# indrajeetadityaroy9/vit-bias-aware-structural-distillation

Measured on AMD Instinct MI355X. Metric: images/sec BASD train step, DeiT-T student / ViT-B teacher bs=256, higher is better.
Workload: dtype bf16

## Files before the change

### include/basd_hip.h

```cpp
#ifndef BASD_HIP_H
#define BASD_HIP_H

#include <stddef.h>
#include <stdint.h>

#ifdef __cplusplus
extern "C" {
#endif

#define BASD_OK 0
#define BASD_ERR_SHAPE 1
#define BASD_ERR_LAUNCH 2
#define BASD_ERR_WORKSPACE 3
#define BASD_ERR_DTYPE 4

#define BASD_STATUS_NONCONVERGED 1
#define BASD_STATUS_NONFINITE 2
#define BASD_STATUS_RANK0 4

#define BASD_DTYPE_F32 0
#define BASD_DTYPE_BF16 1
#define BASD_DTYPE_F64 2

#define BASD_JACOBI_MAX_COLS 256
// ... 30 lines not shown
                    int32_t* status, void* stream);

int basd_mp_rank(const float* evals, int batch, int n, int64_t rows, int d, int cap,
                 int32_t* ranks, int32_t* status, void* stream);

int basd_flag_if_exceeds_f64(const double* values, int64_t n, double tol, int bit, int32_t* status, void* stream);

int basd_angle_weights(const float* sigma, const float* sw, const float* log_temp, int E, int L, int D,
                       int unnormalised, float* d2, float* pre, float* weights, float* coef, void* stream);

int64_t basd_angle_weights_bwd_workspace_bytes(int E, int D, int D_s);
int basd_angle_weights_bwd(const float* g_w, const float* g_pre_out, const float* weights, const float* d2,
                           const float* log_temp, const float* t_seed, const float* v_s, const double* lam_s,
                           const float* proj_s, int E, int L, int D, int D_s, float* g_log_temp, float* w_tok,
                           void* workspace, int64_t workspace_bytes, void* stream);

int64_t basd_selector_frames_workspace_bytes(int n, int D);
int basd_selector_frames(const double* unc, const double* csum, int n, int64_t m_rows, int D, int with_ranks,
                         int32_t* ranks, float* sigma, double* lam, float* v, int32_t* status, void* workspace,
                         int64_t workspace_bytes, void* stream);

int64_t basd_selector_weights_workspace_bytes(int E, int L, int D);
int basd_selector_weights(const float* v_s, const int32_t* ranks, const float* vm_t, const float* sw,
                          const float* log_temp, int E, int L, int D, float* weights, float* pre, float* d2,
                          float* t_seed, int32_t* status, void* workspace, int64_t workspace_bytes, void* stream);

int basd_mix_tokens(const void* const* x_layers, int x_dtype, int L, int E,
                    const float* w, int64_t elems, int64_t per_batch, int64_t batch_stride,
                    float* out, void* stream);

int basd_procrustes_prep(const void* s, int s_dtype, int64_t s_batch_stride, const float* t, const float* imp,
                         int B, int N_s, int N_t, int D_s, int D_t,
                         float* s_w, float* t_w, float* a, float* tr, void* stream);

int basd_mix_grad_dots(const void* const* x_layers, int x_dtype, int L, int E,
                       const float* g, int64_t elems, int64_t per_batch, int64_t batch_stride,
                       double* dots, void* stream);

int basd_bgemm_f64(const void* a, int a_dtype, int64_t a_stride, int lda, int trans_a,
                   const void* b, int b_dtype, int64_t b_stride, int ldb, int trans_b,
                   void* c, int c_dtype, int64_t c_stride, int ldc,
                   int batch, int M, int N, int K, int symmetric, void* stream);
int basd_bgemm_f64_masked(const void* a, int a_dtype, int64_t a_stride, int lda, int trans_a,
                          const void* b, int b_dtype, int64_t b_stride, int ldb, int trans_b,
                          void* c, int c_dtype, int64_t c_stride, int ldc,
                          int batch, int M, int N, int K, int symmetric, const int32_t* skip, void* stream);

int basd_gemm_bf16(const void* x, const void* w, const void* bias, void* y, int64_t M, int N, int K,
                   int epilogue, int tile_run, void* stream);

int basd_gemm_bf16x3_f32(const void* x, const void* w3, float* y, int64_t M, int N, int K, void* stream);

int basd_gemm_bf16_gelu_fwd(const void* x, const void* w, const void* bias, void* pre, void* y, int64_t M, int N,
                            int K, int tile_run, void* stream);
int basd_gemm_bf16_gelu_bwd(const void* dy, const void* wt, const void* pre, void* dpre, int64_t M, int N, int K,
                            int tile_run, void* stream);

int basd_wgrad_bf16(const void* dy, const void* x, int64_t M, int N, int K, float* dw, float* db,
                    void* stream);

int64_t basd_wgrad_workspace_bytes(int64_t M, int N, int K);
int basd_wgrad_bf16_ws(const void* dy, const void* x, int64_t M, int N, int K, float* dw, float* db,
                       void* workspace, int64_t workspace_bytes, void* stream);

int basd_layernorm_fwd_bf16(const void* x, const float* gamma, const float* beta, int64_t rows, int D,
                            float eps, void* y, float* mean, float* rstd, void* stream);
// ... 105 lines not shown
```

### vit-bias-aware-structural-distillation_amd/_native.py

```python
from __future__ import annotations

import contextlib
import ctypes
import os
import subprocess

import torch

_HERE = os.path.dirname(os.path.abspath(__file__))
LIB_PATH = os.environ.get("BASD_LIB") or os.path.join(_HERE, "libbasd_hip.so")
CSRC = os.path.join(_HERE, "csrc")

DTYPE_F32, DTYPE_BF16, DTYPE_F64 = 0, 1, 2
JACOBI_LDS_BYTES = 163840

EXPORTS = (
    "basd_version", "basd_last_error", "basd_token_gram", "basd_token_gram_bf16x3", "basd_gram_f32_centred", "basd_pchol_f64", "basd_jacobi_svd",
    "basd_mp_rank", "basd_flag_if_exceeds_f64", "basd_angle_weights", "basd_ce_uwso",
    "basd_procrustes_workspace_bytes", "basd_procrustes_fwd", "basd_procrustes_bwd_side",
    "basd_procrustes_bwd_workspace_bytes", "basd_procrustes_bwd", "basd_angle_weights_bwd_workspace_bytes",
    "basd_angle_weights_bwd", "basd_mix_tokens", "basd_procrustes_prep", "basd_mix_grad_dots",
    "basd_sf_adamw_step", "basd_lerp", "basd_transpose_bf16_table", "basd_bgemm_f64", "basd_trinv_f64", "basd_bgemm_f64_masked", "basd_trinv_f64_masked", "basd_pchol_f64_masked", "basd_wgrad_bf16", "basd_wgrad_workspace_bytes", "basd_wgrad_bf16_ws", "basd_gemm_bf16",
    "basd_gemm_bf16_gelu_fwd", "basd_gemm_bf16_gelu_bwd", "basd_gemm_bf16x3_f32", "basd_layernorm_fwd_bf16", "basd_layernorm_bwd_bf16",
    "basd_cls_importance_bf16", "basd_add_layernorm_fwd_bf16", "basd_procrustes_bwd_rows", "basd_attention_fwd_bf16", "basd_attention_fwd_qmean_bf16", "basd_attention_bwd_bf16",
    "basd_split_bf16x2_table", "basd_split_patches_bf16x2", "basd_gemm_f32x3", "basd_attention_fwd_f32x3",
    "basd_add_layernorm_fwd_f32", "basd_selector_frames_workspace_bytes", "basd_selector_frames",
    "basd_selector_weights_workspace_bytes", "basd_selector_weights", "basd_attention_fwd_long_bf16",
    "basd_attention_bwd_long_workspace_bytes", "basd_attention_bwd_long_bf16", "basd_attention_fwd_f32x3_long",
    "basd_dwconv7_ln_bf16", "basd_grn_workspace_bytes", "basd_grn_bf16", "basd_patchify_bf16",
    "basd_resample_u8", "basd_ta_normalize_u8", "basd_cls_tally", "basd_resample_u8_packed",
    "basd_mixup_cutmix",
)


_P, _I, _I64, _F, _D = ctypes.c_void_p, ctypes.c_int, ctypes.c_int64, ctypes.c_float, ctypes.c_double
_SIGNATURES = {
    "basd_version": (),
    "basd_last_error": (),
    "basd_token_gram": (_P, _I, _I64, _I, _I, _I64, _P, _I, _P, _P, _P),
    "basd_token_gram_bf16x3": (_P, _I64, _I, _I, _I64, _P, _I, _P, _P, _P),
    "basd_gram_f32_centred": (_P, _I64, _I, _P, _P, _P),
    "basd_pchol_f64": (_P, _I, _I, _D, _P, _P, _I, _P, _P, _P, _P),
    "basd_pchol_f64_masked": (_P, _I, _I, _D, _P, _P, _I, _P, _P, _P, _P, _P),
    "basd_trinv_f64": (_P, _P, _P, _I, _I, _P, _P),
    "basd_trinv_f64_masked": (_P, _P, _P, _I, _I, _P, _P, _P),
    "basd_jacobi_svd": (_P, _I, _I, _I, _I, _I, _F, _I, _I, _P, _P, _P, _I, _P, _P),
    "basd_mp_rank": (_P, _I, _I, _I64, _I, _I, _P, _P, _P),
    "basd_flag_if_exceeds_f64": (_P, _I64, _D, _I, _P, _P),
    "basd_angle_weights": (_P, _P, _P, _I, _I, _I, _I, _P, _P, _P, _P, _P),
    "basd_mix_tokens": (_P, _I, _I, _I, _P, _I64, _I64, _I64, _P, _P),
    "basd_procrustes_prep": (_P, _I, _I64, _P, _P, _I, _I, _I, _I, _I, _P, _P, _P, _P, _P),
    "basd_mix_grad_dots": (_P, _I, _I, _I, _P, _I64, _I64, _I64, _P, _P),
    "basd_procrustes_workspace_bytes": (_I, _I, _I, _I),
    "basd_procrustes_fwd": (_P, _P, _I, _I, _I, _I, _D, _P, _P, _P, _P, _P, _I64, _P),
    "basd_procrustes_bwd_side": (_P, _P, _P, _P, _I, _I, _I, _P, _I, _P, _P),
    "basd_procrustes_bwd_workspace_bytes": (_I, _I),
    "basd_angle_weights_bwd_workspace_bytes": (_I, _I, _I),
    "basd_angle_weights_bwd": (_P, _P, _P, _P, _P, _P, _P, _P, _P, _I, _I, _I, _I, _P, _P, _P, _I64, _P),
    "basd_selector_frames_workspace_bytes": (_I, _I),
    "basd_selector_frames": (_P, _P, _I, _I64, _I, _I, _P, _P, _P, _P, _P, _P, _I64, _P),
    "basd_selector_weights_workspace_bytes": (_I, _I, _I),
    "basd_selector_weights": (_P, _P, _P, _P, _P, _I, _I, _I, _P, _P, _P, _P, _P, _P, _I64, _P),
    "basd_procrustes_bwd": (_P, _P, _P, _P, _P, _P, _I, _I, _I, _I, _P, _I, _P, _P, _P, _I64, _P),
    "basd_ce_uwso": (_P, _P, _P, _I, _I, _F, _P, _P, _P, _P, _P),
    "basd_transpose_bf16_table": (_P, _P, _P, _I, _P),
    "basd_bgemm_f64": (_P, _I, _I64, _I, _I, _P, _I, _I64, _I, _I, _P, _I, _I64, _I, _I, _I, _I, _I, _I, _P),
    "basd_bgemm_f64_masked": (_P, _I, _I64, _I, _I, _P, _I, _I64, _I, _I, _P, _I, _I64, _I, _I, _I, _I, _I, _I, _P, _P),
    "basd_wgrad_bf16": (_P, _P, _I64, _I, _I, _P, _P, _P),
    "basd_wgrad_workspace_bytes": (_I64, _I, _I),
    "basd_wgrad_bf16_ws": (_P, _P, _I64, _I, _I, _P, _P, _P, _I64, _P),
    "basd_gemm_bf16": (_P, _P, _P, _P, _I64, _I, _I, _I, _I, _P),
    "basd_gemm_bf16_gelu_fwd": (_P, _P, _P, _P, _P, _I64, _I, _I, _I, _P),
    "basd_gemm_bf16x3_f32": (_P, _P, _P, _I64, _I, _I, _P),
    "basd_gemm_bf16_gelu_bwd": (_P, _P, _P, _P, _I64, _I, _I, _I, _P),
    "basd_layernorm_fwd_bf16": (_P, _P, _P, _I64, _I, _F, _P, _P, _P, _P),
    "basd_add_layernorm_fwd_bf16": (_P, _P, _P, _P, _I64, _I, _F, _P, _P, _P, _P, _P, _I, _P),
    "basd_layernorm_bwd_bf16": (_P, _P, _P, _P, _P, _I64, _I, _P, _P, _P, _P, _P, _P, _I, _P),
    "basd_procrustes_bwd_rows": (_P, _P, _P, _P, _I64, _I, _I, _P, _I, _P, _P),
    "basd_cls_importance_bf16": (_P, _I, _I, _I, _I, _F, _P, _P),
    "basd_attention_fwd_bf16": (_P, _I, _I, _I, _I, _F, _P, _P, _P, _P),
    "basd_attention_fwd_qmean_bf16": (_P, _I, _I, _I, _I, _F, _P, _P, _P),
    "basd_attention_bwd_bf16": (_P, _P, _P, _P, _I, _I, _I, _I, _F, _P, _P),
    "basd_attention_fwd_long_bf16": (_P, _I, _I, _I, _I, _F, _P, _P, _P, _P, _P),
    "basd_attention_bwd_long_workspace_bytes": (_I, _I, _I, _I),
    "basd_attention_bwd_long_bf16": (_P, _P, _P, _P, _I, _I, _I, _I, _F, _P, _P, _I64, _P),
# ... 438 lines not shown
    dots = torch.zeros(E, L, dtype=torch.float64, device=g.device)
    table = _ptr_table(layers)
    i64 = ctypes.c_int64
    _check(lib().basd_mix_grad_dots(table, code, L, E, _ptr(g.contiguous()), i64(elems), i64(per_batch),
                                    i64(bstride), _ptr(dots), _stream()), "basd_mix_grad_dots")
    return dots


def procrustes_prep(s: torch.Tensor, t: torch.Tensor, imp: torch.Tensor, out=None):
    _need_cuda(s, t, imp)
    if not (s[0].is_contiguous() and s.data_ptr() % 16 == 0):
        s = s.contiguous()
    t = t.contiguous().float()
    imp = imp.contiguous().float()
    B, N_s, D_s = s.shape
    _, N_t, D_t = t.shape
    dev = s.device
    if out is None:
        s_w = torch.empty(B, N_s, D_s, dtype=torch.float32, device=dev)
        t_w = torch.empty(B, N_s, D_t, dtype=torch.float32, device=dev)
        a = torch.empty(B, N_s, dtype=torch.float32, device=dev)
        tr = torch.empty(B, 2, dtype=torch.float32, device=dev)
    else:
        s_w, t_w, a, tr = out
        assert s_w.shape == (B, N_s, D_s) and t_w.shape == (B, N_s, D_t) and a.shape == (B, N_s) and tr.shape == (B, 2)
        for o in out:
            assert o.dtype == torch.float32 and o.is_contiguous()
    _check(lib().basd_procrustes_prep(_ptr(s), _dtype_code(s), ctypes.c_int64(s.stride(0)), _ptr(t), _ptr(imp), B, N_s,
                                      N_t, D_s, D_t, _ptr(s_w), _ptr(t_w), _ptr(a), _ptr(tr), _stream()),
           "basd_procrustes_prep")
    return s_w, t_w, a, tr


def procrustes_bwd_rows(r: torch.Tensor, w: torch.Tensor, a: torch.Tensor, gl: torch.Tensor, out_dtype=torch.float32):
    _need_cuda(r, w, a, gl)
    for t_ in (r, w, a, gl):
        assert t_.dtype == torch.float32 and t_.is_contiguous()
    B, N, D = r.shape
    assert w.shape == r.shape and a.shape == (B, N) and gl.numel() == B
    out = r if out_dtype == torch.float32 else torch.empty(B, N, D, dtype=out_dtype, device=r.device)
    rowdot = torch.empty(B, N, dtype=torch.float32, device=r.device)
    code = DTYPE_F32 if out_dtype == torch.float32 else DTYPE_BF16
    _check(lib().basd_procrustes_bwd_rows(_ptr(r), _ptr(w), _ptr(a), _ptr(gl), ctypes.c_int64(B * N), N, D, _ptr(out),
                                          code, _ptr(rowdot), _stream()), "basd_procrustes_bwd_rows")
    return out, rowdot


def sf_adamw_step(y, g, z, v, *, lr, beta1, beta2, eps, weight_decay, ckp1, bias_correction2) -> None:
    _need_cuda(y, g, z, v)
    n = y.numel()
    assert g.numel() == n and z.numel() == n and v.numel() == n
    for t in (y, g, z, v):
        assert t.dtype == torch.float32 and t.is_contiguous()
    f = ctypes.c_double
    _check(lib().basd_sf_adamw_step(_ptr(y), _ptr(g), _ptr(z), _ptr(v), ctypes.c_int64(n), f(lr), f(beta1),
                                    f(beta2), f(eps), f(weight_decay), f(ckp1), f(bias_correction2), _stream()),
           "basd_sf_adamw_step")


def lerp_(y, z, w: float) -> None:
    _need_cuda(y, z)
    assert y.dtype == torch.float32 and z.dtype == torch.float32 and y.numel() == z.numel()
    _check(lib().basd_lerp(_ptr(y), _ptr(z), ctypes.c_int64(y.numel()), ctypes.c_float(w), _stream()), "basd_lerp")


_SCRATCH: dict = {}
# ... 662 lines not shown
```

### vit-bias-aware-structural-distillation_amd/csrc/stream_kernels.hip

```cpp
#include "basd_common.h"

namespace basd {

constexpr int kMaxE = 8;
constexpr int kMaxL = 64;

struct LayerPtrs { const void* p[kMaxL]; };

template <typename T> struct Vec;
template <> struct Vec<float> {
  static constexpr int N = 4;
  static __device__ __forceinline__ void load(const float* p, float (&v)[4]) {
    const float4 t = *reinterpret_cast<const float4*>(p);
    v[0] = t.x; v[1] = t.y; v[2] = t.z; v[3] = t.w;
  }
};
template <> struct Vec<unsigned short> {
  static constexpr int N = 8;
  static __device__ __forceinline__ void load(const unsigned short* p, float (&v)[8]) {
    const uint4 t = *reinterpret_cast<const uint4*>(p);
    const unsigned int w[4] = {t.x, t.y, t.z, t.w};
#pragma unroll
    for (int i = 0; i < 4; ++i) {
      v[2 * i] = __uint_as_float(w[i] << 16);
// ... 331 lines not shown
      for (int k = 0; k < 32; ++k) {
        const float4 p = *reinterpret_cast<const float4*>(s_part + ((sb * 32 + k) * 64 + 4 * cq));
        m.x += p.x; m.y += p.y; m.z += p.z; m.w += p.w;
      }
      *reinterpret_cast<float4*>(s_mu + sb * 64 + 4 * cq) = m;
    }
    __syncthreads();
    if (act) {
      const float4 mu = *reinterpret_cast<const float4*>(s_mu + sb * 64 + 4 * cq);
      float* dst = is_s ? sw : tw;
      const int D = is_s ? D_s : D_t;
      float acc = 0.f;
#pragma unroll
      for (int i = 0; i < TPT; ++i) {
        const int n = tg + 32 * i;
        if (n < N_s) {
          const float ra = s_ra[n];
          const float4 v = make_float4(ra * (x[i].x - mu.x), ra * (x[i].y - mu.y), ra * (x[i].z - mu.z), ra * (x[i].w - mu.w));
          *reinterpret_cast<float4*>(dst + (size_t)n * D + col) = v;
          acc = fmaf(v.x, v.x, fmaf(v.y, v.y, fmaf(v.z, v.z, fmaf(v.w, v.w, acc))));
        }
      }
      if (is_s) trs += (double)acc; else trt += (double)acc;
    }
  }
  trs = wave_sum_d(trs); trt = wave_sum_d(trt);
  __syncthreads();
  if ((tid & 63) == 0) { s_red[tid >> 6] = (float)trs; s_red[32 + (tid >> 6)] = (float)trt; }
  __syncthreads();
  if (tid == 0) {
    float x = 0.f, y = 0.f;
    for (int w = 0; w < (nt >> 6); ++w) { x += s_red[w]; y += s_red[32 + w]; }
    tr_all[(size_t)b * 2] = x; tr_all[(size_t)b * 2 + 1] = y;
  }
}

template <typename TO>
__global__ __launch_bounds__(256) void procrustes_bwd_rows_kernel(const float* __restrict__ p, const float* __restrict__ w,
                                                                  const float* __restrict__ a, const float* __restrict__ gl,
                                                                  int64_t rows, int rows_per_batch, int D, TO* out,
                                                                  float* __restrict__ rowdot) {
  const int lane = threadIdx.x & 63, wave = threadIdx.x >> 6;
  const int nq = D >> 2;
  for (int64_t row = (int64_t)blockIdx.x * 4 + wave; row < rows; row += (int64_t)gridDim.x * 4) {
    const float c2 = 2.f * gl[row / rows_per_batch];
    const float c = c2 * sqrtf(a[row]);
    const float4* p4 = reinterpret_cast<const float4*>(p + row * D);
    const float4* w4 = reinterpret_cast<const float4*>(w + row * D);
    float dot = 0.f;
    for (int q = lane; q < nq; q += 64) {
      const float4 pv = p4[q], wv = w4[q];
      const float4 rv = make_float4(wv.x - pv.x, wv.y - pv.y, wv.z - pv.z, wv.w - pv.w);
      dot = fmaf(rv.x, wv.x, fmaf(rv.y, wv.y, fmaf(rv.z, wv.z, fmaf(rv.w, wv.w, dot))));
      if constexpr (sizeof(TO) == 4) {
        reinterpret_cast<float4*>(out + row * D)[q] = make_float4(c * rv.x, c * rv.y, c * rv.z, c * rv.w);
      } else {
        __hip_bfloat16 b0 = __float2bfloat16(c * rv.x), b1 = __float2bfloat16(c * rv.y);
        __hip_bfloat16 b2 = __float2bfloat16(c * rv.z), b3 = __float2bfloat16(c * rv.w);
        uint2 o;
        o.x = (unsigned int)(*reinterpret_cast<unsigned short*>(&b0)) | ((unsigned int)(*reinterpret_cast<unsigned short*>(&b1)) << 16);
        o.y = (unsigned int)(*reinterpret_cast<unsigned short*>(&b2)) | ((unsigned int)(*reinterpret_cast<unsigned short*>(&b3)) << 16);
        reinterpret_cast<uint2*>(out + row * D)[q] = o;
      }
    }
    dot = wave_sum(dot);
    if (lane == 0) rowdot[row] = c2 * dot;
// ... 226 lines not shown
  const bool vec_ok = D_s % 4 == 0 && D_t % 4 == 0 && s_batch_stride % 4 == 0 && ((uintptr_t)s & 15) == 0 &&
                      ((uintptr_t)t & 15) == 0 && ((uintptr_t)s_w & 15) == 0 && ((uintptr_t)t_w & 15) == 0 && lds4 <= 64 * 1024;
  if (vec_ok && (s_dtype == BASD_DTYPE_F32 || s_dtype == BASD_DTYPE_BF16) && D_s % 64 == 0 && D_t % 64 == 0 && N_s <= 256) {
    const size_t lds5 = ((size_t)4 * ((N_s + 3) & ~3) + 2 * 32 * 64 + 2 * 64 + 64) * 4;
#define BASD_PREP5(TS, TPT)                                                                                  \
  hipLaunchKernelGGL((procrustes_prep_v5_kernel<TS, TPT>), dim3(B), dim3(1024), lds5, st, (const TS*)s, t, imp, N_s, N_t, \
                     D_s, D_t, s_batch_stride, s_w, t_w, a, tr)
    if (s_dtype == BASD_DTYPE_F32) { if (N_s <= 224) BASD_PREP5(float, 7); else BASD_PREP5(float, 8); }
    else { if (N_s <= 224) BASD_PREP5(unsigned short, 7); else BASD_PREP5(unsigned short, 8); }
#undef BASD_PREP5
    return check_launch("procrustes_prep (single pass)");
  }
  if (vec_ok && (s_dtype == BASD_DTYPE_F32 || s_dtype == BASD_DTYPE_BF16)) {
    if (s_dtype == BASD_DTYPE_F32)
      hipLaunchKernelGGL(procrustes_prep_v4_kernel<float>, dim3(B), dim3(1024), lds4, st, (const float*)s, t, imp,
                         N_s, N_t, D_s, D_t, s_batch_stride, s_w, t_w, a, tr);
    else
      hipLaunchKernelGGL(procrustes_prep_v4_kernel<unsigned short>, dim3(B), dim3(1024), lds4, st,
                         (const unsigned short*)s, t, imp, N_s, N_t, D_s, D_t, s_batch_stride, s_w, t_w, a, tr);
    return check_launch("procrustes_prep (vectorised)");
  }
  if (s_dtype == BASD_DTYPE_F32) {
    hipLaunchKernelGGL(procrustes_prep_kernel<float>, dim3(B), dim3(512), lds, st, (const float*)s, t, imp,
                       N_s, N_t, D_s, D_t, s_batch_stride, s_w, t_w, a, tr);
  } else if (s_dtype == BASD_DTYPE_BF16) {
    hipLaunchKernelGGL(procrustes_prep_kernel<unsigned short>, dim3(B), dim3(512), lds, st,
                       (const unsigned short*)s, t, imp, N_s, N_t, D_s, D_t, s_batch_stride, s_w, t_w, a, tr);
  } else {
    return fail(BASD_ERR_DTYPE, "procrustes_prep: dtype %d", s_dtype);
  }
  return check_launch("procrustes_prep");
}

extern "C" int basd_procrustes_bwd_rows(const float* r, const float* w, const float* a, const float* gl, int64_t rows,
                                        int rows_per_batch, int D, void* out, int out_dtype, float* rowdot,
                                        void* stream) {
  using namespace basd;
  if (rows <= 0) return BASD_OK;
  if (D < 4 || D % 4 || rows_per_batch < 1) return fail(BASD_ERR_SHAPE, "procrustes_bwd_rows: D=%d rows_per_batch=%d", D, rows_per_batch);
  int64_t grid = (rows + 3) / 4;
  if (grid > 4096) grid = 4096;
  hipStream_t st = (hipStream_t)stream;
  if (out_dtype == BASD_DTYPE_F32)
    hipLaunchKernelGGL(procrustes_bwd_rows_kernel<float>, dim3((int)grid), dim3(256), 0, st, r, w, a, gl, rows,
                       rows_per_batch, D, (float*)out, rowdot);
  else if (out_dtype == BASD_DTYPE_BF16)
    hipLaunchKernelGGL(procrustes_bwd_rows_kernel<unsigned short>, dim3((int)grid), dim3(256), 0, st, r, w, a, gl, rows,
                       rows_per_batch, D, (unsigned short*)out, rowdot);
  else
    return fail(BASD_ERR_DTYPE, "procrustes_bwd_rows: out dtype %d", out_dtype);
  return check_launch("procrustes_bwd_rows");
}
```

### vit-bias-aware-structural-distillation_amd/losses/combined.py

```python
from __future__ import annotations

import torch
import torch.nn as nn
import torch.nn.functional as F

from . import functional as BF
from .layer_selector import GrassmannianLayerSelector


def _align_token_count(tokens: torch.Tensor, target_n: int) -> torch.Tensor:
    if tokens.shape[1] == target_n:
        return tokens
    r = BF.resample_matrix(tokens.shape[1], target_n, tokens.device, tokens.dtype)
    return torch.matmul(r, tokens)


class _CeUwsoFn(torch.autograd.Function):

    @staticmethod
    def forward(ctx, logits, geo, targets, smoothing):
        out4, dl = BF.get_ops().ce_uwso(logits, targets, smoothing, geo)
        ctx.save_for_backward(dl, out4)
        ctx.mark_non_differentiable(out4)
        return out4[0], out4
# ... 7 lines not shown
class _MixImportanceFn(torch.autograd.Function):

    @staticmethod
    def forward(ctx, weights, imp):
        ctx.save_for_backward(weights, imp)
        return torch.einsum("el,lbn->ebn", weights, imp)

    @staticmethod
    def backward(ctx, g):
        weights, imp = ctx.saved_tensors
        g_w = g_imp = None
        if ctx.needs_input_grad[0]:
            g_w = torch.bmm(g.permute(1, 0, 2), imp.permute(1, 2, 0)).sum(dim=0).to(weights.dtype)
        if ctx.needs_input_grad[1]:
            g_imp = torch.einsum("el,ebn->lbn", weights, g)
        return g_w, g_imp


class BASDLoss(nn.Module):
    def __init__(self, base_criterion: nn.Module, student_dim: int, teacher_dim: int,
                 student_depth: int, num_student_tokens: int, *, config, teacher_has_cls_token: bool):
        super().__init__()
        self.base_criterion = base_criterion
        self.teacher_has_cls_token = teacher_has_cls_token
        self.num_student_tokens = num_student_tokens
        n_pts = config.num_extraction_points
        if n_pts == 1:
            self.token_layers = [student_depth - 1]
        else:
            self.token_layers = [round(i * (student_depth - 1) / (n_pts - 1)) for i in range(n_pts)]
        self.layer_selector = GrassmannianLayerSelector(
            num_extraction_points=len(self.token_layers), student_dim=student_dim, teacher_dim=teacher_dim)
        self.last_terms: dict[str, torch.Tensor] = {}

    def _fused_ce(self, student_output, targets) -> bool:
        c = self.base_criterion
        return (type(c) is nn.CrossEntropyLoss and c.weight is None and c.reduction == "mean"
                and student_output.dim() == 2 and student_output.dtype == torch.float32
                and BF.get_ops().handles(student_output)
                and (targets.dim() == 2 or (targets.dim() == 1 and c.ignore_index < 0)))

    def forward(self, student_output, targets, student_intermediates, all_teacher_tokens, all_teacher_attns):
        fused_ce = self._fused_ce(student_output, targets)
        ce_loss = None if fused_ce else self.base_criterion(student_output, targets)

        sel = self.layer_selector
        weights, teacher_indices = sel.mixing_weights(student_intermediates, all_teacher_tokens, self.token_layers)
        mixed = BF.mix_layers(weights, [all_teacher_tokens[j] for j in teacher_indices])
        imp = torch.stack([BF.importance_from_attention(all_teacher_attns[j], self.teacher_has_cls_token)
                           for j in teacher_indices])
        mixed_imp = _MixImportanceFn.apply(weights, imp)

        students = []
        for layer_idx in self.token_layers:
            s = student_intermediates[layer_idx]
            if s.shape[1] != self.num_student_tokens:
                raise ValueError(f"student layer {layer_idx} has {s.shape[1]} tokens, expected {self.num_student_tokens}")
            students.append(s)
        geo_each = BF.procrustes_all(students, mixed, mixed_imp).mean(dim=1)
        geo_loss = geo_each.mean()
        if fused_ce:
            total, out4 = _CeUwsoFn.apply(student_output, geo_loss.float(), targets, float(self.base_criterion.label_smoothing))
            self.last_terms = {"ce": out4[1], "geo": geo_each.detach()}
            return total

        eps = torch.finfo(ce_loss.dtype).eps
        inv = torch.stack([1.0 / ce_loss.detach().clamp(min=eps), 1.0 / geo_loss.detach().float().clamp(min=eps)])
        w = inv / inv.sum()
        self.last_terms = {"ce": ce_loss.detach(), "geo": geo_each.detach()}
        return w[0] * ce_loss + w[1] * geo_loss
```

### vit-bias-aware-structural-distillation_amd/losses/functional.py

```python
from __future__ import annotations

import torch
import torch.nn.functional as F

from ._ops import get_ops, note_library_gemm

_EPS32 = float(torch.finfo(torch.float32).eps)
PCHOL_TOL = 1e-13


class BasdShapeError(NotImplementedError):
    pass


PROCRUSTES_BWD_FUSED = __import__("os").environ.get("BASD_PROCRUSTES_BWD", "fused") != "lib"
WIDE_PANEL = 192
WIDE_BLOCK = 96
WIDE_COS_TOL = 1e-4
WIDE_DIRECT_SWEEPS = 8
_ROUND_CACHE: dict = {}


def _wide_sweeps(nblk: int) -> int:
    return 3 + (nblk + 1) // 2 if nblk > 4 else 4
# ... 375 lines not shown
class _MixFn(torch.autograd.Function):
    @staticmethod
    def forward(ctx, w, *layers):
        ops = get_ops()
        ctx.layers = layers
        return ops.mix_tokens(list(layers), w.detach().float())

    @staticmethod
    def backward(ctx, g):
        ops = get_ops()
        dots = ops.mix_grad_dots(list(ctx.layers), g.contiguous().float())
        return (dots.float(), *([None] * len(ctx.layers)))


def mix_layers(w: torch.Tensor, layers) -> torch.Tensor:
    return _MixFn.apply(w, *[t.detach() for t in layers])


class _ProcrustesFn(torch.autograd.Function):

    @staticmethod
    def forward(ctx, t_all, imp_all, *students):
        ops = get_ops()
        E = len(students)
        n_s, n_t = students[0].shape[1], t_all.shape[2]
        b, d_s, d_t, dev = students[0].shape[0], students[0].shape[2], t_all.shape[3], t_all.device
        s_w = torch.empty(E * b, n_s, d_s, dtype=torch.float32, device=dev)
        t_w = torch.empty(E * b, n_s, d_t, dtype=torch.float32, device=dev)
        a = torch.empty(E * b, n_s, dtype=torch.float32, device=dev)
        tr = torch.empty(E * b, 2, dtype=torch.float32, device=dev)
        for i in range(E):
            sl = slice(i * b, (i + 1) * b)
            ops.procrustes_prep(students[i], t_all[i], imp_all[i], out=(s_w[sl], t_w[sl], a[sl], tr[sl]))
        ctx.token_side = n_s <= d_s
        if not ops.jacobi_fits(min(n_s, d_s), min(n_s, d_s)):
            raise BasdShapeError(f"Procrustes core min(N_s, D_s) = {min(n_s, d_s)} does not fit the LDS-resident Jacobi")
        nuc, fac_s, a_t = ops.procrustes_fwd(s_w, t_w, PCHOL_TOL)
        ctx.save_for_backward(s_w, t_w, a, imp_all, fac_s, a_t)
        ctx.n_t, ctx.E = n_t, E
        ctx.s_dtype = students[0].dtype
        return (tr[:, 0] + tr[:, 1] - 2.0 * nuc).view(E, -1)

    @staticmethod
    def backward(ctx, g_loss):
        s_w, t_w, a, imp_all, *polar = ctx.saved_tensors
        E = ctx.E
        n_s, n_t = s_w.shape[1], ctx.n_t
        ops = get_ops()
        gl = g_loss.float().reshape(-1).contiguous()
        if PROCRUSTES_BWD_FUSED and getattr(ops, "procrustes_bwd_supported", None) is not None and \
                ops.procrustes_bwd_supported(n_s, s_w.shape[2], t_w.shape[2]) and ctx.s_dtype in (torch.float32, torch.bfloat16):
            g_s, g_t, g_a = ops.procrustes_bwd(s_w, t_w, a, gl, polar[0].contiguous(), polar[1].contiguous(), ctx.s_dtype)
        else:
            note_library_gemm("Procrustes backward: fp32 bmm (A_t t_w)")
            if ctx.token_side:
                p_s, p_t = polar[0] @ s_w, polar[1] @ t_w
            else:
                p_s = polar[0].clone() if ctx.s_dtype == torch.float32 else polar[0]
                p_t = polar[1] @ t_w
            g_s, dot_s = ops.procrustes_bwd_rows(p_s, s_w, a, gl, out_dtype=ctx.s_dtype)
            g_t, dot_t = ops.procrustes_bwd_rows(p_t, t_w, a, gl, out_dtype=torch.float32)
            g_a = (dot_s + dot_t) / (2.0 * a)
        imp = imp_all.float().reshape(-1, n_t)
        if n_t != n_s:
            r = resample_matrix(n_t, n_s, s_w.device)
            tot = (imp @ r.t()).sum(-1, keepdim=True)
            g_raw = (g_a - (a * g_a).sum(-1, keepdim=True)) / tot
            g_imp = g_raw @ r
            g_t = torch.matmul(r.t(), g_t)
        else:
            tot = imp.sum(-1, keepdim=True)
            g_imp = (g_a - (a * g_a).sum(-1, keepdim=True)) / tot
        b = g_s.shape[0] // E
        return (g_t.view(E, b, n_t, -1), g_imp.view(E, b, n_t), *g_s.view(E, b, n_s, -1).unbind(0))


def procrustes_all(students, t_all: torch.Tensor, imp_all: torch.Tensor) -> torch.Tensor:
    return _ProcrustesFn.apply(t_all.contiguous().float(), imp_all.contiguous().float(), *students)


def procrustes(s: torch.Tensor, t: torch.Tensor, imp: torch.Tensor) -> torch.Tensor:
    return procrustes_all([s], t.unsqueeze(0), imp.unsqueeze(0))[0]
```

Baseline: 8015.

## Fuse teacher layer mixing into Procrustes prep kernel

Adds a fused HIP kernel that computes the weighted mix of teacher layers directly inside the Procrustes preparation step. The mixed teacher tensor is never written to and re-read from global memory, and the per-student prep launches become a single launch. The backward pass reuses the existing grad-dots kernel for the mixing weights. This adds a more complex kernel with register-heavy templating and a fallback path for shapes it does not support.

```diff
diff --git a/include/basd_hip.h b/include/basd_hip.h
--- a/include/basd_hip.h
+++ b/include/basd_hip.h
@@ -86,6 +86,11 @@
 int basd_procrustes_prep(const void* s, int s_dtype, int64_t s_batch_stride, const float* t, const float* imp,
                          int B, int N_s, int N_t, int D_s, int D_t,
                          float* s_w, float* t_w, float* a, float* tr, void* stream);
+
+int basd_mix_procrustes_prep(const void* const* x_layers, int x_dtype, int L, int E, const float* w,
+                             int64_t layer_batch_stride, const void* const* students, int s_dtype,
+                             int64_t s_batch_stride, const float* imp, int B, int N, int D_s, int D_t,
+                             float* s_w, float* t_w, float* a, float* tr, void* stream);
 
 int basd_mix_grad_dots(const void* const* x_layers, int x_dtype, int L, int E,
                        const float* g, int64_t elems, int64_t per_batch, int64_t batch_stride,
diff --git a/vit-bias-aware-structural-distillation_amd/_native.py b/vit-bias-aware-structural-distillation_amd/_native.py
--- a/vit-bias-aware-structural-distillation_amd/_native.py
+++ b/vit-bias-aware-structural-distillation_amd/_native.py
@@ -29,7 +29,7 @@
     "basd_attention_bwd_long_workspace_bytes", "basd_attention_bwd_long_bf16", "basd_attention_fwd_f32x3_long",
     "basd_dwconv7_ln_bf16", "basd_grn_workspace_bytes", "basd_grn_bf16", "basd_patchify_bf16",
     "basd_resample_u8", "basd_ta_normalize_u8", "basd_cls_tally", "basd_resample_u8_packed",
-    "basd_mixup_cutmix",
+    "basd_mixup_cutmix", "basd_mix_procrustes_prep",
 )
 
 
@@ -51,6 +51,7 @@
     "basd_mix_tokens": (_P, _I, _I, _I, _P, _I64, _I64, _I64, _P, _P),
     "basd_procrustes_prep": (_P, _I, _I64, _P, _P, _I, _I, _I, _I, _I, _P, _P, _P, _P, _P),
     "basd_mix_grad_dots": (_P, _I, _I, _I, _P, _I64, _I64, _I64, _P, _P),
+    "basd_mix_procrustes_prep": (_P, _I, _I, _I, _P, _I64, _P, _I, _I64, _P, _I, _I, _I, _I, _P, _P, _P, _P, _P),
     "basd_procrustes_workspace_bytes": (_I, _I, _I, _I),
     "basd_procrustes_fwd": (_P, _P, _I, _I, _I, _I, _D, _P, _P, _P, _P, _P, _I64, _P),
     "basd_procrustes_bwd_side": (_P, _P, _P, _P, _I, _I, _I, _P, _I, _P, _P),
@@ -555,6 +556,62 @@
     return s_w, t_w, a, tr
 
 
+MIX_PREP_MAX_TOKENS = 224
+MIX_PREP_MAX_E, MIX_PREP_MAX_L = 8, 64
+
+
+def _mix_prep_dense(t: torch.Tensor) -> bool:
+    return (t.dim() == 3 and t.stride(2) == 1 and t.stride(1) == t.shape[2] and t.stride(0) % 8 == 0
+            and t.data_ptr() % 16 == 0)
+
+
+def mix_procrustes_prep_supported(layers, students, imp_all=None) -> bool:
+    layers, students = list(layers), list(students)
+    if not (2 <= len(layers) <= MIX_PREP_MAX_L and 1 <= len(students) <= MIX_PREP_MAX_E):
+        return False
+    t0, s0 = layers[0], students[0]
+    ok_dtype = (torch.float32, torch.bfloat16)
+    if t0.dim() != 3 or s0.dim() != 3 or t0.dtype not in ok_dtype or s0.dtype not in ok_dtype:
+        return False
+    if any(t.shape != t0.shape or t.dtype != t0.dtype or t.stride(0) != t0.stride(0) or not _mix_prep_dense(t)
+           for t in layers):
+        return False
+    if any(s.shape != s0.shape or s.dtype != s0.dtype or s.stride(0) != s0.stride(0) or not _mix_prep_dense(s)
+           for s in students):
+        return False
+    b, n, d_t = t0.shape
+    if s0.shape[0] != b or s0.shape[1] != n or not 1 <= n <= MIX_PREP_MAX_TOKENS:
+        return False
+    if d_t % 64 or s0.shape[2] % 64 or b < 1:
+        return False
+    return imp_all is None or tuple(imp_all.shape) == (len(students), b, n)
+
+
+def mix_procrustes_prep(layers, w: torch.Tensor, students, imp_all: torch.Tensor):
+    layers, students = list(layers), list(students)
+    _need_cuda(*layers, *students, w, imp_all)
+    if not mix_procrustes_prep_supported(layers, students, imp_all):
+        raise BasdNativeError("mix_procrustes_prep: unsupported shapes / layouts (ask mix_procrustes_prep_supported; "
+                              "mix_tokens + procrustes_prep take everything else)")
+    E, L = len(students), len(layers)
+    assert tuple(w.shape) == (E, L)
+    b, n, d_t = layers[0].shape
+    d_s = students[0].shape[2]
+    w = w.detach().contiguous().float()
+    imp_all = imp_all.detach().contiguous().float()
+    dev = w.device
+    s_w = torch.empty(E * b, n, d_s, dtype=torch.float32, device=dev)
+    t_w = torch.empty(E * b, n, d_t, dtype=torch.float32, device=dev)
+    a = torch.empty(E * b, n, dtype=torch.float32, device=dev)
+    tr = torch.empty(E * b, 2, dtype=torch.float32, device=dev)
+    i64 = ctypes.c_int64
+    _check(lib().basd_mix_procrustes_prep(_ptr_table(layers), _dtype_code(layers[0]), L, E, _ptr(w),
+                                          i64(layers[0].stride(0)), _ptr_table(students), _dtype_code(students[0]),
+                                          i64(students[0].stride(0)), _ptr(imp_all), b, n, d_s, d_t, _ptr(s_w), _ptr(t_w),
+                                          _ptr(a), _ptr(tr), _stream()), "basd_mix_procrustes_prep")
+    return s_w, t_w, a, tr
+
+
 def procrustes_bwd_rows(r: torch.Tensor, w: torch.Tensor, a: torch.Tensor, gl: torch.Tensor, out_dtype=torch.float32):
     _need_cuda(r, w, a, gl)
     for t_ in (r, w, a, gl):
diff --git a/vit-bias-aware-structural-distillation_amd/csrc/stream_kernels.hip b/vit-bias-aware-structural-distillation_amd/csrc/stream_kernels.hip
--- a/vit-bias-aware-structural-distillation_amd/csrc/stream_kernels.hip
+++ b/vit-bias-aware-structural-distillation_amd/csrc/stream_kernels.hip
@@ -387,6 +387,193 @@
     float x = 0.f, y = 0.f;
     for (int w = 0; w < (nt >> 6); ++w) { x += s_red[w]; y += s_red[32 + w]; }
     tr_all[(size_t)b * 2] = x; tr_all[(size_t)b * 2 + 1] = y;
+  }
+}
+
+constexpr int kFusedE = 4;
+struct StudentPtrs { const void* p[kFusedE]; };
+
+template <typename TL> struct RawQuad;
+template <> struct RawQuad<float> {
+  using type = float4;
+  static __device__ __forceinline__ type zero() { return make_float4(0.f, 0.f, 0.f, 0.f); }
+  static __device__ __forceinline__ float4 widen(const type& v) { return v; }
+};
+template <> struct RawQuad<unsigned short> {
+  using type = uint2;
+  static __device__ __forceinline__ type zero() { return make_uint2(0u, 0u); }
+  static __device__ __forceinline__ float4 widen(const type& v) {
+    return make_float4(__uint_as_float(v.x << 16), __uint_as_float(v.x & 0xffff0000u),
+                       __uint_as_float(v.y << 16), __uint_as_float(v.y & 0xffff0000u));
+  }
+};
+
+template <typename TL, typename TS, int E, int TPT>
+__global__ __launch_bounds__(512) void mix_procrustes_prep_kernel(
+    LayerPtrs layers, int L, const float* __restrict__ w, int64_t t_batch_stride, StudentPtrs studs,
+    int64_t s_batch_stride, const float* __restrict__ imp_all, int B, int N, int D_s, int D_t,
+    float* __restrict__ sw_all, float* __restrict__ tw_all, float* __restrict__ a_all, float* __restrict__ tr_all) {
+  using Raw = typename RawQuad<TL>::type;
+  constexpr int kRawRegs = TPT <= 2 ? 64 : (E > 2 ? 28 : 56);
+  constexpr int LC = kRawRegs / (TPT * (sizeof(TL) == 2 ? 2 : 4));
+  static_assert(LC >= 1, "no room for one layer's loads");
+  extern __shared__ __align__(16) float sm[];
+  const int n4 = (N + 3) & ~3;
+  float* s_a = sm;
+  float* s_ra = s_a + E * n4;
+  float* s_part = s_ra + E * n4;
+  float* s_mu = s_part + E * 32 * 64;
+  float* s_red = s_mu + E * 64;
+  const int b = blockIdx.x, tid = threadIdx.x, nt = blockDim.x;
+
+#pragma unroll
+  for (int e = 0; e < E; ++e) {
+    const float* imp = imp_all + ((size_t)e * B + b) * N;
+    float part = 0.f;
+    for (int n = tid; n < N; n += nt) {
+      const float v = imp[n];
+      s_a[e * n4 + n] = v;
+      part += v;
+    }
+    part = wave_sum(part);
+    if ((tid & 63) == 0) s_red[e * 32 + (tid >> 6)] = part;
+  }
+  __syncthreads();
+#pragma unroll
+  for (int e = 0; e < E; ++e) {
+    float tot = 0.f;
+    for (int wv = 0; wv < (nt >> 6); ++wv) tot += s_red[e * 32 + wv];
+    for (int n = tid; n < N; n += nt) {
+      const float an = s_a[e * n4 + n] / tot;
+      s_a[e * n4 + n] = an;
+      s_ra[e * n4 + n] = sqrtf(an);
+      a_all[((size_t)e * B + b) * N + n] = an;
+    }
+  }
+  __syncthreads();
+  const int tg = tid >> 4, cq = tid & 15;
+  const int G_s = D_s >> 6, G = G_s + (D_t >> 6);
+  double tr_cur[E][2], tr_oth[E][2];
+#pragma unroll
+  for (int e = 0; e < E; ++e) { tr_cur[e][0] = tr_cur[e][1] = 0.0; tr_oth[e][0] = tr_oth[e][1] = 0.0; }
+  for (int g = 0; g < G; ++g) {
+    const bool is_s = g < G_s;
+    const int col = (is_s ? 64 * g : 64 * (g - G_s)) + 4 * cq;
+    float4 x[E][TPT];
+#pragma unroll
+    for (int e = 0; e < E; ++e)
+#pragma unroll
+      for (int i = 0; i < TPT; ++i) x[e][i] = make_float4(0.f, 0.f, 0.f, 0.f);
+    if (is_s) {
+#pragma unroll
+      for (int e = 0; e < E; ++e) {
+        const TS* s = static_cast<const TS*>(studs.p[e]) + (size_t)b * s_batch_stride;
+#pragma unroll
+        for (int i = 0; i < TPT; ++i) {
+          const int n = tg + 32 * i;
+          if (n < N) x[e][i] = load_quad<TS>(s + (size_t)n * D_s + col);
+        }
+      }
+    } else {
+      const size_t base = (size_t)b * t_batch_stride + col;
+      for (int j0 = 0; j0 < L; j0 += LC) {
+        Raw raw[LC][TPT];
+#pragma unroll
+        for (int jj = 0; jj < LC; ++jj) {
+#pragma unroll
+          for (int i = 0; i < TPT; ++i) raw[jj][i] = RawQuad<TL>::zero();
+          if (j0 + jj < L) {
+            const TL* p = static_cast<const TL*>(layers.p[j0 + jj]) + base;
+#pragma unroll
+            for (int i = 0; i < TPT; ++i) {
+              const int n = tg + 32 * i;
+              if (n < N) raw[jj][i] = *reinterpret_cast<const Raw*>(p + (size_t)n * D_t);
+            }
+          }
+        }
+#pragma unroll
+        for (int jj = 0; jj < LC; ++jj) {
+          if (j0 + jj < L) {
+#pragma unroll
+            for (int e = 0; e < E; ++e) {
+              const float wij = w[e * L + j0 + jj];
+#pragma unroll
+              for (int i = 0; i < TPT; ++i) {
+                const float4 r = RawQuad<TL>::widen(raw[jj][i]);
+                x[e][i].x = fmaf(wij, r.x, x[e][i].x); x[e][i].y = fmaf(wij, r.y, x[e][i].y);
+                x[e][i].z = fmaf(wij, r.z, x[e][i].z); x[e][i].w = fmaf(wij, r.w, x[e][i].w);
+              }
+            }
+          }
+        }
+      }
+    }
+#pragma unroll
+    for (int e = 0; e < E; ++e) {
+      float4 acc = make_float4(0.f, 0.f, 0.f, 0.f);
+#pragma unroll
+      for (int i = 0; i < TPT; ++i) {
+        const int n = tg + 32 * i;
+        if (n < N) {
+          const float an = s_a[e * n4 + n];
+          acc.x = fmaf(an, x[e][i].x, acc.x); acc.y = fmaf(an, x[e][i].y, acc.y);
+          acc.z = fmaf(an, x[e][i].z, acc.z); acc.w = fmaf(an, x[e][i].w, acc.w);
+        }
+      }
+      *reinterpret_cast<float4*>(s_part + ((e * 32 + tg) * 64 + 4 * cq)) = acc;
+    }
+    lds_barrier();
+    if (tg < E) {
+      float4 m = make_float4(0.f, 0.f, 0.f, 0.f);
+#pragma unroll 4
+      for (int k = 0; k < 32; ++k) {
+        const float4 p = *reinterpret_cast<const float4*>(s_part + ((tg * 32 + k) * 64 + 4 * cq));
+        m.x += p.x; m.y += p.y; m.z += p.z; m.w += p.w;
+      }
+      *reinterpret_cast<float4*>(s_mu + tg * 64 + 4 * cq) = m;
+    }
+    lds_barrier();
+#pragma unroll
+    for (int e = 0; e < E; ++e) {
+      const float4 mu = *reinterpret_cast<const float4*>(s_mu + e * 64 + 4 * cq);
+      const int D = is_s ? D_s : D_t;
+      float* dst = (is_s ? sw_all : tw_all) + ((size_t)e * B + b) * N * D;
+      float acc = 0.f;
+#pragma unroll
+      for (int i = 0; i < TPT; ++i) {
+        const int n = tg + 32 * i;
+        if (n < N) {
+          const float ra = s_ra[e * n4 + n];
+          const float4 v = make_float4(ra * (x[e][i].x - mu.x), ra * (x[e][i].y - mu.y), ra * (x[e][i].z - mu.z), ra * (x[e][i].w - mu.w));
+          *reinterpret_cast<float4*>(dst + (size_t)n * D + col) = v;
+          acc = fmaf(v.x, v.x, fmaf(v.y, v.y, fmaf(v.z, v.z, fmaf(v.w, v.w, acc))));
+        }
+      }
+      if (is_s) tr_cur[e][0] += (double)acc; else tr_cur[e][1] += (double)acc;
+    }
+#pragma unroll
+    for (int e = 0; e < E; ++e)
+#pragma unroll
+      for (int k = 0; k < 2; ++k) { const double t_ = tr_cur[e][k]; tr_cur[e][k] = tr_oth[e][k]; tr_oth[e][k] = t_; }
+  }
+  const bool odd = (G & 1) != 0;
+  __syncthreads();
+#pragma unroll
+  for (int e = 0; e < E; ++e)
+#pragma unroll
+    for (int k = 0; k < 2; ++k) {
+      const double r0 = wave_sum_d(odd ? tr_oth[e][k] : tr_cur[e][k]);
+      const double r1 = wave_sum_d(odd ? tr_cur[e][k] : tr_oth[e][k]);
+      if ((tid & 63) == 0) {
+        s_red[(e * 2 + k) * 16 + (tid >> 6)] = (float)r0;
+        s_red[(e * 2 + k) * 16 + 8 + (tid >> 6)] = (float)r1;
+      }
+    }
+  __syncthreads();
+  if (tid < 2 * E) {
+    float v = 0.f;
+    for (int wv = 0; wv < 16; ++wv) v += s_red[tid * 16 + wv];
+    tr_all[((size_t)(tid >> 1) * B + b) * 2 + (tid & 1)] = v;
   }
 }
 
@@ -679,6 +866,84 @@
   return check_launch("procrustes_prep");
 }
 
+namespace basd {
+
+constexpr int kFusedTPT = 7, kFusedShortTPT = 2;
+
+template <typename TL, typename TS, int E>
+static void launch_mix_prep(const void* const* layers, int L, const float* w, int64_t t_bs, const void* const* students,
+                            int64_t s_bs, const float* imp, int B, int N, int D_s, int D_t, float* s_w, float* t_w,
+                            float* a, float* tr, hipStream_t st) {
+  LayerPtrs lp;
+  for (int i = 0; i < kMaxL; ++i) lp.p[i] = i < L ? layers[i] : nullptr;
+  StudentPtrs sp;
+  for (int i = 0; i < kFusedE; ++i) sp.p[i] = i < E ? students[i] : nullptr;
+  const size_t lds = ((size_t)2 * E * ((N + 3) & ~3) + (size_t)E * (32 * 64 + 64 + 32)) * 4;
+  if (N <= 32 * kFusedShortTPT)
+    hipLaunchKernelGGL((mix_procrustes_prep_kernel<TL, TS, E, kFusedShortTPT>), dim3(B), dim3(512), lds, st, lp, L, w,
+                       t_bs, sp, s_bs, imp, B, N, D_s, D_t, s_w, t_w, a, tr);
+  else
+    hipLaunchKernelGGL((mix_procrustes_prep_kernel<TL, TS, E, kFusedTPT>), dim3(B), dim3(512), lds, st, lp, L, w, t_bs,
+                       sp, s_bs, imp, B, N, D_s, D_t, s_w, t_w, a, tr);
+}
+
+template <typename TL, typename TS>
+static void dispatch_mix_prep(int E, const void* const* layers, int L, const float* w, int64_t t_bs,
+                              const void* const* students, int64_t s_bs, const float* imp, int B, int N, int D_s,
+                              int D_t, float* s_w, float* t_w, float* a, float* tr, hipStream_t st) {
+  switch (E) {
+    case 1: launch_mix_prep<TL, TS, 1>(layers, L, w, t_bs, students, s_bs, imp, B, N, D_s, D_t, s_w, t_w, a, tr, st); break;
+    case 2: launch_mix_prep<TL, TS, 2>(layers, L, w, t_bs, students, s_bs, imp, B, N, D_s, D_t, s_w, t_w, a, tr, st); break;
+    case 3: launch_mix_prep<TL, TS, 3>(layers, L, w, t_bs, students, s_bs, imp, B, N, D_s, D_t, s_w, t_w, a, tr, st); break;
+    default: launch_mix_prep<TL, TS, 4>(layers, L, w, t_bs, students, s_bs, imp, B, N, D_s, D_t, s_w, t_w, a, tr, st); break;
+  }
+}
+
+}
+
+extern "C" int basd_mix_procrustes_prep(const void* const* x_layers, int x_dtype, int L, int E, const float* w,
+                                        int64_t layer_batch_stride, const void* const* students, int s_dtype,
+                                        int64_t s_batch_stride, const float* imp, int B, int N, int D_s, int D_t,
+                                        float* s_w, float* t_w, float* a, float* tr, void* stream) {
+  using namespace basd;
+  if (B <= 0) return BASD_OK;
+  if (L < 1 || L > kMaxL) return fail(BASD_ERR_SHAPE, "mix_procrustes_prep: L=%d out of 1..%d", L, kMaxL);
+  if (E < 1 || E > kMaxE) return fail(BASD_ERR_SHAPE, "mix_procrustes_prep: E=%d out of 1..%d", E, kMaxE);
+  if (N < 1 || N > 32 * kFusedTPT || D_s < 64 || D_t < 64 || D_s % 64 || D_t % 64)
+    return fail(BASD_ERR_SHAPE, "mix_procrustes_prep: N=%d (1..%d), D_s=%d, D_t=%d (multiples of 64)", N, 32 * kFusedTPT,
+                D_s, D_t);
+  if ((x_dtype != BASD_DTYPE_F32 && x_dtype != BASD_DTYPE_BF16) || (s_dtype != BASD_DTYPE_F32 && s_dtype != BASD_DTYPE_BF16))
+    return fail(BASD_ERR_DTYPE, "mix_procrustes_prep: dtypes %d / %d", x_dtype, s_dtype);
+  const uintptr_t t_mask = x_dtype == BASD_DTYPE_F32 ? 15 : 7, s_mask = s_dtype == BASD_DTYPE_F32 ? 15 : 7;
+  if (layer_batch_stride < (int64_t)N * D_t || layer_batch_stride % 4 || s_batch_stride < (int64_t)N * D_s || s_batch_stride % 4)
+    return fail(BASD_ERR_SHAPE, "mix_procrustes_prep: batch strides %lld / %lld", (long long)layer_batch_stride,
+                (long long)s_batch_stride);
+  for (int j = 0; j < L; ++j)
+    if (!x_layers[j] || ((uintptr_t)x_layers[j] & t_mask)) return fail(BASD_ERR_SHAPE, "mix_procrustes_prep: layer %d misaligned", j);
+  for (int e = 0; e < E; ++e)
+    if (!students[e] || ((uintptr_t)students[e] & s_mask)) return fail(BASD_ERR_SHAPE, "mix_procrustes_prep: student %d misaligned", e);
+  if (((uintptr_t)s_w & 15) || ((uintptr_t)t_w & 15)) return fail(BASD_ERR_SHAPE, "mix_procrustes_prep: outputs misaligned");
+  hipStream_t st = (hipStream_t)stream;
+  for (int e0 = 0; e0 < E; e0 += kFusedE) {
+    const int Ec = E - e0 < kFusedE ? E - e0 : kFusedE;
+    const float* wc = w + (size_t)e0 * L;
+    const float* ic = imp + (size_t)e0 * B * N;
+    float* swc = s_w + (size_t)e0 * B * N * D_s;
+    float* twc = t_w + (size_t)e0 * B * N * D_t;
+    float* ac = a + (size_t)e0 * B * N;
+    float* trc = tr + (size_t)e0 * B * 2;
+#define BASD_MIXPREP(TL, TS) \
+  dispatch_mix_prep<TL, TS>(Ec, x_layers, L, wc, layer_batch_stride, students + e0, s_batch_stride, ic, B, N, D_s, D_t, swc, twc, ac, trc, st)
+    if (x_dtype == BASD_DTYPE_BF16) {
+      if (s_dtype == BASD_DTYPE_BF16) BASD_MIXPREP(unsigned short, unsigned short); else BASD_MIXPREP(unsigned short, float);
+    } else {
+      if (s_dtype == BASD_DTYPE_BF16) BASD_MIXPREP(float, unsigned short); else BASD_MIXPREP(float, float);
+    }
+#undef BASD_MIXPREP
+  }
+  return check_launch("mix_procrustes_prep");
+}
+
 extern "C" int basd_procrustes_bwd_rows(const float* r, const float* w, const float* a, const float* gl, int64_t rows,
                                         int rows_per_batch, int D, void* out, int out_dtype, float* rowdot,
                                         void* stream) {
diff --git a/vit-bias-aware-structural-distillation_amd/losses/combined.py b/vit-bias-aware-structural-distillation_amd/losses/combined.py
--- a/vit-bias-aware-structural-distillation_amd/losses/combined.py
+++ b/vit-bias-aware-structural-distillation_amd/losses/combined.py
@@ -63,6 +63,7 @@
         self.layer_selector = GrassmannianLayerSelector(
             num_extraction_points=len(self.token_layers), student_dim=student_dim, teacher_dim=teacher_dim)
         self.last_terms: dict[str, torch.Tensor] = {}
+        self.fused_mix_prep = str(getattr(config, "fused_mix_prep", True)).lower() in ("1", "true")
 
     def _fused_ce(self, student_output, targets) -> bool:
         c = self.base_criterion
@@ -77,7 +78,7 @@
 
         sel = self.layer_selector
         weights, teacher_indices = sel.mixing_weights(student_intermediates, all_teacher_tokens, self.token_layers)
-        mixed = BF.mix_layers(weights, [all_teacher_tokens[j] for j in teacher_indices])
+        layers = [all_teacher_tokens[j] for j in teacher_indices]
         imp = torch.stack([BF.importance_from_attention(all_teacher_attns[j], self.teacher_has_cls_token)
                            for j in teacher_indices])
         mixed_imp = _MixImportanceFn.apply(weights, imp)
@@ -88,7 +89,7 @@
             if s.shape[1] != self.num_student_tokens:
                 raise ValueError(f"student layer {layer_idx} has {s.shape[1]} tokens, expected {self.num_student_tokens}")
             students.append(s)
-        geo_each = BF.procrustes_all(students, mixed, mixed_imp).mean(dim=1)
+        geo_each = BF.mix_procrustes(weights, layers, students, mixed_imp, fused=self.fused_mix_prep).mean(dim=1)
         geo_loss = geo_each.mean()
         if fused_ce:
             total, out4 = _CeUwsoFn.apply(student_output, geo_loss.float(), targets, float(self.base_criterion.label_smoothing))
diff --git a/vit-bias-aware-structural-distillation_amd/losses/functional.py b/vit-bias-aware-structural-distillation_amd/losses/functional.py
--- a/vit-bias-aware-structural-distillation_amd/losses/functional.py
+++ b/vit-bias-aware-structural-distillation_amd/losses/functional.py
@@ -431,47 +431,89 @@
         for i in range(E):
             sl = slice(i * b, (i + 1) * b)
             ops.procrustes_prep(students[i], t_all[i], imp_all[i], out=(s_w[sl], t_w[sl], a[sl], tr[sl]))
-        ctx.token_side = n_s <= d_s
-        if not ops.jacobi_fits(min(n_s, d_s), min(n_s, d_s)):
-            raise BasdShapeError(f"Procrustes core min(N_s, D_s) = {min(n_s, d_s)} does not fit the LDS-resident Jacobi")
-        nuc, fac_s, a_t = ops.procrustes_fwd(s_w, t_w, PCHOL_TOL)
-        ctx.save_for_backward(s_w, t_w, a, imp_all, fac_s, a_t)
-        ctx.n_t, ctx.E = n_t, E
-        ctx.s_dtype = students[0].dtype
-        return (tr[:, 0] + tr[:, 1] - 2.0 * nuc).view(E, -1)
+        return _procrustes_values(ctx, ops, s_w, t_w, a, tr, imp_all, E, n_t, students[0].dtype)
 
     @staticmethod
     def backward(ctx, g_loss):
-        s_w, t_w, a, imp_all, *polar = ctx.saved_tensors
-        E = ctx.E
-        n_s, n_t = s_w.shape[1], ctx.n_t
+        return _procrustes_grads(ctx, g_loss)
+
+
+def _procrustes_values(ctx, ops, s_w, t_w, a, tr, imp_all, E, n_t, s_dtype):
+    n_s, d_s = s_w.shape[1], s_w.shape[2]
+    ctx.token_side = n_s <= d_s
+    if not ops.jacobi_fits(min(n_s, d_s), min(n_s, d_s)):
+        raise BasdShapeError(f"Procrustes core min(N_s, D_s) = {min(n_s, d_s)} does not fit the LDS-resident Jacobi")
+    nuc, fac_s, a_t = ops.procrustes_fwd(s_w, t_w, PCHOL_TOL)
+    ctx.save_for_backward(s_w, t_w, a, imp_all, fac_s, a_t)
+    ctx.n_t, ctx.E = n_t, E
+    ctx.s_dtype = s_dtype
+    return (tr[:, 0] + tr[:, 1] - 2.0 * nuc).view(E, -1)
+
+
+def _procrustes_grads(ctx, g_loss):
+    s_w, t_w, a, imp_all, *polar = ctx.saved_tensors
+    E = ctx.E
+    n_s, n_t = s_w.shape[1], ctx.n_t
+    ops = get_ops()
+    gl = g_loss.float().reshape(-1).contiguous()
+    if PROCRUSTES_BWD_FUSED and getattr(ops, "procrustes_bwd_supported", None) is not None and \
+            ops.procrustes_bwd_supported(n_s, s_w.shape[2], t_w.shape[2]) and ctx.s_dtype in (torch.float32, torch.bfloat16):
+        g_s, g_t, g_a = ops.procrustes_bwd(s_w, t_w, a, gl, polar[0].contiguous(), polar[1].contiguous(), ctx.s_dtype)
+    else:
+        note_library_gemm("Procrustes backward: fp32 bmm (A_t t_w)")
+        if ctx.token_side:
+            p_s, p_t = polar[0] @ s_w, polar[1] @ t_w
+        else:
+            p_s = polar[0].clone() if ctx.s_dtype == torch.float32 else polar[0]
+            p_t = polar[1] @ t_w
+        g_s, dot_s = ops.procrustes_bwd_rows(p_s, s_w, a, gl, out_dtype=ctx.s_dtype)
+        g_t, dot_t = ops.procrustes_bwd_rows(p_t, t_w, a, gl, out_dtype=torch.float32)
+        g_a = (dot_s + dot_t) / (2.0 * a)
+    imp = imp_all.float().reshape(-1, n_t)
+    if n_t != n_s:
+        r = resample_matrix(n_t, n_s, s_w.device)
+        tot = (imp @ r.t()).sum(-1, keepdim=True)
+        g_raw = (g_a - (a * g_a).sum(-1, keepdim=True)) / tot
+        g_imp = g_raw @ r
+        g_t = torch.matmul(r.t(), g_t)
+    else:
+        tot = imp.sum(-1, keepdim=True)
+        g_imp = (g_a - (a * g_a).sum(-1, keepdim=True)) / tot
+    b = g_s.shape[0] // E
+    return (g_t.view(E, b, n_t, -1), g_imp.view(E, b, n_t), *g_s.view(E, b, n_s, -1).unbind(0))
+
+
+class _MixProcrustesFn(torch.autograd.Function):
+
+    @staticmethod
+    def forward(ctx, w, imp_all, n_layers, *tensors):
         ops = get_ops()
-        gl = g_loss.float().reshape(-1).contiguous()
-        if PROCRUSTES_BWD_FUSED and getattr(ops, "procrustes_bwd_supported", None) is not None and \
-                ops.procrustes_bwd_supported(n_s, s_w.shape[2], t_w.shape[2]) and ctx.s_dtype in (torch.float32, torch.bfloat16):
-            g_s, g_t, g_a = ops.procrustes_bwd(s_w, t_w, a, gl, polar[0].contiguous(), polar[1].contiguous(), ctx.s_dtype)
-        else:
-            note_library_gemm("Procrustes backward: fp32 bmm (A_t t_w)")
-            if ctx.token_side:
-                p_s, p_t = polar[0] @ s_w, polar[1] @ t_w
-            else:
-                p_s = polar[0].clone() if ctx.s_dtype == torch.float32 else polar[0]
-                p_t = polar[1] @ t_w
-            g_s, dot_s = ops.procrustes_bwd_rows(p_s, s_w, a, gl, out_dtype=ctx.s_dtype)
-            g_t, dot_t = ops.procrustes_bwd_rows(p_t, t_w, a, gl, out_dtype=torch.float32)
-            g_a = (dot_s + dot_t) / (2.0 * a)
-        imp = imp_all.float().reshape(-1, n_t)
-        if n_t != n_s:
-            r = resample_matrix(n_t, n_s, s_w.device)
-            tot = (imp @ r.t()).sum(-1, keepdim=True)
-            g_raw = (g_a - (a * g_a).sum(-1, keepdim=True)) / tot
-            g_imp = g_raw @ r
-            g_t = torch.matmul(r.t(), g_t)
-        else:
-            tot = imp.sum(-1, keepdim=True)
-            g_imp = (g_a - (a * g_a).sum(-1, keepdim=True)) / tot
-        b = g_s.shape[0] // E
-        return (g_t.view(E, b, n_t, -1), g_imp.view(E, b, n_t), *g_s.view(E, b, n_s, -1).unbind(0))
+        layers, students = tensors[:n_layers], tensors[n_layers:]
+        ctx.layers = layers
+        s_w, t_w, a, tr = ops.mix_procrustes_prep(list(layers), w.detach().float(), list(students), imp_all)
+        return _procrustes_values(ctx, ops, s_w, t_w, a, tr, imp_all, len(students), layers[0].shape[1], students[0].dtype)
+
+    @staticmethod
+    def backward(ctx, g_loss):
+        g_t, g_imp, *g_s = _procrustes_grads(ctx, g_loss)
+        dots = get_ops().mix_grad_dots(list(ctx.layers), g_t.contiguous().float())
+        return (dots.float(), g_imp, None, *([None] * len(ctx.layers)), *g_s)
+
+
+def mix_procrustes_supported(layers, students) -> bool:
+    ops = get_ops()
+    supported = getattr(ops, "mix_procrustes_prep_supported", None)
+    return supported is not None and bool(supported([t.detach() for t in layers], [s.detach() for s in students]))
+
+
+def mix_procrustes_all(w: torch.Tensor, layers, students, imp_all: torch.Tensor) -> torch.Tensor:
+    return _MixProcrustesFn.apply(w, imp_all.contiguous().float(), len(layers), *[t.detach() for t in layers], *students)
+
+
+def mix_procrustes(w: torch.Tensor, layers, students, imp_all: torch.Tensor, fused: bool = True) -> torch.Tensor:
+    if fused and mix_procrustes_supported(layers, students):
+        return mix_procrustes_all(w, layers, students, imp_all)
+    return procrustes_all(students, mix_layers(w, layers), imp_all)
 
 
 def procrustes_all(students, t_all: torch.Tensor, imp_all: torch.Tensor) -> torch.Tensor:
```

Result: no change. 8008 (-0.1%).
